# um-dsrg/Super-Resolution-Meta-Attention-Networks

Measured on AMD Instinct MI355X. Metric: LR-patches/sec (128x128x3, x4) fwd+bwd, higher is better.
Workload: dtype f32

## Files before the change

super-resolution-meta-attention-networks_amd/csrc/wgrad3x3_mfma.hip:

```cpp
#include "sisr_common.h"
#include <string.h>
#include <stdlib.h>

#define WT_H 8
#define WT_W 32
#define WH_H (WT_H + 2)
#define WH_W (WT_W + 2)
#define WSTR 32
#define X_ITEMS (WH_H * WH_W * 8)
#define X_ITERS ((X_ITEMS + 255) / 256)
#define Y_ITEMS (WT_H * WT_W * 8)
#define Y_ITERS (Y_ITEMS / 256)
#define LDS_X (WH_H * WH_W * WSTR)
#define LDS_Y (WT_H * WT_W * WSTR)
#define SLAB (9 * 16 * 64)
#define WG_MAX_UNITS 64

struct WgradParams {
  const float* x;
  View xv;
  const float* dy;
  View yv;
  const float* dy_scale;
  const float* dy_shift;
// ... 100 lines not shown
          const int ghe = h0 - 1 + er;
          if (!interior && !refl) e = sisr_keep_if(e, ghe >= 0 && ghe < H && gwe >= 0 && gwe < W);
          if (tl < 160) *reinterpret_cast<f32x4*>(ldx + er * (WH_W * WSTR) + (eside ? WH_W - 1 : 0) * WSTR + ec4 * 4) = e;
        }
      }
    }
    __syncthreads();

#pragma unroll 1
    for (int r = 2 * wave; r < 2 * wave + 2; ++r) {
      const float* xa = ldx + (r * WH_W + kk) * WSTR + i;
      const float* yb = ldy + (r * WT_W + kk) * WSTR + i;
#pragma unroll 4
      for (int u = 0; u < 16; ++u) {
        const float bv = yb[u * 2 * WSTR];
        float av[9];
#pragma unroll
        for (int t = 0; t < 9; ++t) av[t] = xa[((t / 3) * WH_W + (t % 3) + 2 * u) * WSTR];
#pragma unroll
        for (int t = 0; t < 9; ++t) acc[t] = __builtin_amdgcn_mfma_f32_32x32x2f32(av[t], bv, acc[t], 0, 0, 0);
      }
    }
  }

  __syncthreads();
  float* red = lds;
  if (wave >= 2) {
#pragma unroll
    for (int t = 0; t < 9; ++t)
#pragma unroll
      for (int r = 0; r < 16; ++r) red[(wave - 2) * SLAB + (t * 16 + r) * 64 + lane] = acc[t][r];
  }
  __syncthreads();
  if (wave < 2) {
#pragma unroll
    for (int t = 0; t < 9; ++t)
#pragma unroll
      for (int r = 0; r < 16; ++r) acc[t][r] += red[wave * SLAB + (t * 16 + r) * 64 + lane];
  }
  __syncthreads();
  if (wave == 1) {
#pragma unroll
    for (int t = 0; t < 9; ++t)
#pragma unroll
      for (int r = 0; r < 16; ++r) red[(t * 16 + r) * 64 + lane] = acc[t][r];
  }
  if (do_bias) *reinterpret_cast<f32x4*>(red + SLAB + tid * 4) = bsum;
  __syncthreads();
  if (wave == 0) {
    float* out = p.slabs + ((long)blockIdx.x * nrows + blockIdx.y) * SLAB;
#pragma unroll
    for (int t = 0; t < 9; ++t)
#pragma unroll
      for (int r = 0; r < 16; ++r) out[(t * 16 + r) * 64 + lane] = acc[t][r] + red[(t * 16 + r) * 64 + lane];
  }
  if (do_bias && tid < 32) {
    float s = 0.f;
    const int c4 = tid >> 2, e = tid & 3;
    for (int k = 0; k < 32; ++k) s += red[SLAB + (k * 8 + c4) * 4 + e];
    p.bias_slabs[((long)blockIdx.x * p.cout_chunks * 2 + cq * 2 + coh) * 32 + tid] = s;
  }
}

__global__ __launch_bounds__(256, 2) void wgrad3x3_c64_kernel(WgradParams p) { wgrad3x3_c64_body(p); }
__global__ __launch_bounds__(256, 2) void wgrad3x3_c64_geo_kernel(WgradParams p) { wgrad3x3_c64_body<true>(p); }

#define WG_BATCH 8
struct WgradBatch {
  WgradParams job[WG_BATCH];
};
__global__ __launch_bounds__(256, 2) void wgrad3x3_c64_batch_kernel(WgradBatch bt) { wgrad3x3_c64_body(bt.job[blockIdx.z]); }
__global__ __launch_bounds__(256, 2) void wgrad3x3_c64_geo_batch_kernel(WgradBatch bt) { wgrad3x3_c64_body<true>(bt.job[blockIdx.z]); }

#define FW_X (WH_H * WH_W * 64)
#define FW_Y (WT_H * WT_W * 64)

template <bool GEO = false>
static __device__ __forceinline__ void wgrad3x3_c64_full_body(const WgradParams& p) {
  extern __shared__ __attribute__((aligned(16))) float lds[];
  float* ldx = lds;
  float* ldy = lds + FW_X;
  const int tid = threadIdx.x, lane = tid & 63, wave = tid >> 6;
  const int pair = blockIdx.y;
  const int cq = pair % p.cout_chunks, cc = pair / p.cout_chunks;
  const int cih = __builtin_amdgcn_readfirstlane(wave >> 1), coh = __builtin_amdgcn_readfirstlane(wave & 1);
  const int i = lane & 31, kk = lane >> 5;
  const int H = p.H, W = p.W;
  const bool do_bias = p.bias_slabs && cc == 0;
  const bool affine = p.dy_scale != nullptr || p.dy_shift != nullptr;
  const int Cout = p.cout_chunks * 64;

  f32x16 acc[9];
#pragma unroll
  for (int t = 0; t < 9; ++t) acc[t] = (f32x16){0};
  f32x4 bsa = {0.f, 0.f, 0.f, 0.f}, bsb = bsa;

  const int tiles_per_img = p.tiles_w * p.tiles_h;
  const int total = tiles_per_img * p.B;
  int t_begin = blockIdx.x, t_end = total, t_step = p.S;
  if ((p.S & 7) == 0) {
    const int xcd = blockIdx.x & 7, idx = blockIdx.x >> 3, per = (total + 7) >> 3;
    t_begin = xcd * per + idx;
    t_end = min(total, (xcd + 1) * per);
    t_step = p.S >> 3;
  }
  struct Stage {
    f32x4 x[WH_H][2];
    f32x4 xe[2];
    f32x4 y[WT_H][2];
  };
  Stage st;
  const int c8 = tid & 7, pcol = tid >> 3;
  const int eidx = tid % 160, er = eidx >> 4, eside = (eidx >> 3) & 1, ec8 = eidx & 7;
  auto decode = [&](int tile, int& b, int& h0, int& w0) {
    b = tile / tiles_per_img;
    const int tr = tile - b * tiles_per_img;
    const int th = tr / p.tiles_w;
    h0 = th * WT_H;
    w0 = (tr - th * p.tiles_w) * WT_W;
  };
  const bool refl = GEO && p.geo_reflect;
  const int gup = GEO ? p.geo_up : 0, ysub = GEO ? p.geo_ysub : 0;
  auto xpix = [&](int g, int n) {
    if (refl) g = g < 0 ? -g : (g >= n ? 2 * n - 2 - g : g);
    return min(max(g, 0), n - 1) >> gup;
  };
  auto issue = [&](int tile) {
    int b, h0, w0;
    decode(tile, b, h0, w0);
    const sisr_rsrc_t rx = sisr_rsrc(p.x + (long)b * p.xv.sB + p.xv.chunk(cc));
    const sisr_rsrc_t ry = sisr_rsrc(p.dy + (long)b * p.yv.sB + p.yv.chunk(cq));
    const unsigned vx = (unsigned)(xpix(w0 + pcol, W) * (int)p.xv.sW + c8 * 8) * 4u;
    const unsigned vy = (unsigned)((min(w0 + pcol, W - 1) >> ysub) * (int)p.yv.sW + c8 * 8) * 4u;
#pragma unroll
    for (int r = 0; r < WH_H; ++r) {
      const unsigned so = (unsigned)(xpix(h0 - 1 + r, H) * (int)p.xv.sH) * 4u;
      st.x[r][0] = sisr_buf_load4(rx, vx, so);
      st.x[r][1] = sisr_buf_load4(rx, vx + 16u, so);
    }
    {
      const int gwe = xpix(eside ? w0 + WT_W : w0 - 1, W);
      const unsigned ve = (unsigned)(xpix(h0 - 1 + er, H) * (int)p.xv.sH + gwe * (int)p.xv.sW + ec8 * 8) * 4u;
      st.xe[0] = sisr_buf_load4(rx, ve, 0u);
      st.xe[1] = sisr_buf_load4(rx, ve + 16u, 0u);
    }
#pragma unroll
    for (int r = 0; r < WT_H; ++r) {
      const unsigned so = (unsigned)((min(h0 + r, H - 1) >> ysub) * (int)p.yv.sH) * 4u;
      st.y[r][0] = sisr_buf_load4(ry, vy, so);
      st.y[r][1] = sisr_buf_load4(ry, vy + 16u, so);
    }
  };
  auto commit = [&](int tile) {
    int b, h0, w0;
    decode(tile, b, h0, w0);
    const bool interior = !ysub && h0 >= 1 && h0 + WT_H + 1 <= H && w0 >= 1 && w0 + WT_W + 1 <= W;
    const bool okc = w0 + pcol < W;
    const bool oky = okc && !(ysub && ((w0 + pcol) & 1));
    float* lx = ldx + (pcol + 1) * 64 + c8 * 8;
    if (!interior && !refl) {
#pragma unroll
      for (int r = 0; r < WH_H; ++r) {
        const int gh = h0 - 1 + r;
        const bool ok = gh >= 0 && gh < H && okc;
        st.x[r][0] = sisr_keep_if(st.x[r][0], ok);
        st.x[r][1] = sisr_keep_if(st.x[r][1], ok);
      }
      const int gwe = eside ? w0 + WT_W : w0 - 1, ghe = h0 - 1 + er;
      const bool oke = ghe >= 0 && ghe < H && gwe >= 0 && gwe < W;
      st.xe[0] = sisr_keep_if(st.xe[0], oke);
      st.xe[1] = sisr_keep_if(st.xe[1], oke);
    }
#pragma unroll
    for (int r = 0; r < WH_H; ++r) {
      *reinterpret_cast<f32x4*>(lx + r * (WH_W * 64)) = st.x[r][0];
      *reinterpret_cast<f32x4*>(lx + r * (WH_W * 64) + 4) = st.x[r][1];
    }
    if (tid < 160) {
      float* le = ldx + (er * WH_W + (eside ? WH_W - 1 : 0)) * 64 + ec8 * 8;
      *reinterpret_cast<f32x4*>(le) = st.xe[0];
      *reinterpret_cast<f32x4*>(le + 4) = st.xe[1];
    }
    if (affine) {
      f32x4 s4a = {1.f, 1.f, 1.f, 1.f}, s4b = s4a, t4a = {0.f, 0.f, 0.f, 0.f}, t4b = t4a;
      if (p.dy_scale) {
        const float* sp = p.dy_scale + (long)b * Cout + cq * 64 + c8 * 8;
        s4a = *reinterpret_cast<const f32x4*>(sp);
        s4b = *reinterpret_cast<const f32x4*>(sp + 4);
      }
      if (p.dy_shift) {
        const float* tp = p.dy_shift + (long)b * Cout + cq * 64 + c8 * 8;
        t4a = *reinterpret_cast<const f32x4*>(tp);
        t4b = *reinterpret_cast<const f32x4*>(tp + 4);
      }
#pragma unroll
      for (int r = 0; r < WT_H; ++r) {
        st.y[r][0] = st.y[r][0] * s4a + t4a;
        st.y[r][1] = st.y[r][1] * s4b + t4b;
      }
    }
    if (!interior) {
#pragma unroll
      for (int r = 0; r < WT_H; ++r) {
        const bool ok = oky && (h0 + r < H) && !(ysub && ((h0 + r) & 1));
        st.y[r][0] = sisr_keep_if(st.y[r][0], ok);
        st.y[r][1] = sisr_keep_if(st.y[r][1], ok);
      }
    }
    float* ly = ldy + pcol * 64 + c8 * 8;
#pragma unroll
    for (int r = 0; r < WT_H; ++r) {
      *reinterpret_cast<f32x4*>(ly + r * (WT_W * 64)) = st.y[r][0];
      *reinterpret_cast<f32x4*>(ly + r * (WT_W * 64) + 4) = st.y[r][1];
    }
    if (do_bias) {
#pragma unroll
      for (int r = 0; r < WT_H; ++r) {
        bsa += st.y[r][0];
        bsb += st.y[r][1];
      }
    }
  };

  if (t_begin < t_end) {
    issue(t_begin);
    commit(t_begin);
  }
  __syncthreads();
  for (int tile = t_begin; tile < t_end; tile += t_step) {
    const bool has_next = tile + t_step < t_end;
    if (has_next) issue(tile + t_step);
    {
      const float* xa = ldx + kk * 64 + cih * 32 + i;
      const float* yb = ldy + kk * 64 + coh * 32 + i;
      float bv = yb[0], av[9];
#pragma unroll
      for (int t = 0; t < 9; ++t) av[t] = xa[((t / 3) * WH_W + (t % 3)) * 64];
#pragma unroll 1
      for (int r = 0; r < WT_H; ++r) {
        const int rn = r + 1 < WT_H ? 1 : 0;
        const float* xn = xa + rn * (WH_W * 64);
        const float* yn = yb + rn * (WT_W * 64);
#pragma unroll
        for (int u = 0; u < 16; ++u) {
          float bn, an[9];
          if (u < 15) {
            bn = yb[(u + 1) * 2 * 64];
#pragma unroll
            for (int t = 0; t < 9; ++t) an[t] = xa[((t / 3) * WH_W + (t % 3) + 2 * (u + 1)) * 64];
          } else {
            bn = yn[0];
#pragma unroll
            for (int t = 0; t < 9; ++t) an[t] = xn[((t / 3) * WH_W + (t % 3)) * 64];
          }
          __builtin_amdgcn_sched_barrier(0);
#pragma unroll
          for (int t = 0; t < 9; ++t) acc[t] = __builtin_amdgcn_mfma_f32_32x32x2f32(av[t], bv, acc[t], 0, 0, 0);
          __builtin_amdgcn_sched_barrier(0);
          bv = bn;
#pragma unroll
          for (int t = 0; t < 9; ++t) av[t] = an[t];
        }
        xa = xn;
        yb = yn;
      }
    }
    __syncthreads();
    if (has_next) {
      commit(tile + t_step);
      __syncthreads();
    }
  }

  {
    float* out = p.slabs + ((long)blockIdx.x * ((long)gridDim.y * 4) + pair * 4 + cih * 2 + coh) * SLAB;
#pragma unroll
    for (int t = 0; t < 9; ++t)
#pragma unroll
      for (int r = 0; r < 16; ++r) out[(t * 16 + r) * 64 + lane] = acc[t][r];
  }
  if (do_bias) {
    __syncthreads();
    float* red = lds;
    *reinterpret_cast<f32x4*>(red + tid * 8) = bsa;
    *reinterpret_cast<f32x4*>(red + tid * 8 + 4) = bsb;
    __syncthreads();
    if (tid < 64) {
      const int cc8 = tid >> 3, e = tid & 7;
      float s = 0.f;
      for (int k = 0; k < 32; ++k) s += red[(k * 8 + cc8) * 8 + e];
      p.bias_slabs[((long)blockIdx.x * p.cout_chunks + cq) * 64 + tid] = s;
    }
  }
}

__global__ __launch_bounds__(256, 1) void wgrad3x3_c64_full_kernel(WgradParams p) { wgrad3x3_c64_full_body(p); }
__global__ __launch_bounds__(256, 1) void wgrad3x3_c64_full_batch_kernel(WgradBatch bt) { wgrad3x3_c64_full_body(bt.job[blockIdx.z]); }
__global__ __launch_bounds__(256, 1) void wgrad3x3_c64_full_geo_kernel(WgradParams p) { wgrad3x3_c64_full_body<true>(p); }

#define W4_TH 4
#define W4_HH (W4_TH + 2)
#define W4G_X (W4_HH * WH_W * 64)
#define W4G_Y (W4_TH * WT_W * 64)
#define W4G_CHUNK (4 * 32 * 64)
#define W4G_LDS ((W4G_X + W4G_Y + 2 * W4G_CHUNK) * 4)

__global__ __launch_bounds__(256, 1) void wgrad3x3_c64_w4_kernel(WgradParams p) {
  extern __shared__ __attribute__((aligned(16))) float lds[];
  float* const ldx = lds;
  float* const ldy = lds + W4G_X;
  float* const vch = ldy + W4G_Y;
  float* const mch = vch + W4G_CHUNK;
  const int tid = threadIdx.x, lane = tid & 63, wave = tid >> 6;
  const int pair = blockIdx.y;
  const int cq = pair % p.cout_chunks, cc = pair / p.cout_chunks;
  const int cih = __builtin_amdgcn_readfirstlane(wave >> 1), coh = __builtin_amdgcn_readfirstlane(wave & 1);
  const int i = lane & 31, kk = lane >> 5;
  const int H = p.H, W = p.W;
  const bool do_bias = p.bias_slabs && cc == 0;
  const bool affine = p.dy_scale != nullptr || p.dy_shift != nullptr;
  const int Cout = p.cout_chunks * 64;

  f32x16 acc[16];
#pragma unroll
  for (int t = 0; t < 16; ++t) acc[t] = (f32x16){0};
  f32x4 bsa = {0.f, 0.f, 0.f, 0.f}, bsb = bsa;

  const int tiles_w = p.tiles_w, tiles_h = (H + W4_TH - 1) / W4_TH;
  const int tiles_per_img = tiles_w * tiles_h;
  const int total = tiles_per_img * p.B;
  int t_begin = blockIdx.x, t_end = total, t_step = p.S;
  if ((p.S & 7) == 0) {
    const int xcd = blockIdx.x & 7, idx = blockIdx.x >> 3, per = (total + 7) >> 3;
    t_begin = xcd * per + idx;
    t_end = min(total, (xcd + 1) * per);
    t_step = p.S >> 3;
  }
  struct Stage {
    f32x4 x[W4_HH][2];
    f32x4 xe[2];
    f32x4 y[W4_TH][2];
  };
  Stage st;
  const int c8 = tid & 7, pcol = tid >> 3;
  const int eidx = tid % 96, er = eidx >> 4, eside = (eidx >> 3) & 1, ec8 = eidx & 7;
  auto decode = [&](int tile, int& b, int& h0, int& w0) {
    b = tile / tiles_per_img;
    const int tr = tile - b * tiles_per_img;
    const int th = tr / tiles_w;
    h0 = th * W4_TH;
    w0 = (tr - th * tiles_w) * WT_W;
  };
  auto issue = [&](int tile) {
    int b, h0, w0;
    decode(tile, b, h0, w0);
    const sisr_rsrc_t rx = sisr_rsrc(p.x + (long)b * p.xv.sB + p.xv.chunk(cc));
    const sisr_rsrc_t ry = sisr_rsrc(p.dy + (long)b * p.yv.sB + p.yv.chunk(cq));
    const unsigned vx = (unsigned)(min(w0 + pcol, W - 1) * (int)p.xv.sW + c8 * 8) * 4u;
    const unsigned vy = (unsigned)(min(w0 + pcol, W - 1) * (int)p.yv.sW + c8 * 8) * 4u;
#pragma unroll
    for (int r = 0; r < W4_HH; ++r) {
      const unsigned so = (unsigned)(min(max(h0 - 1 + r, 0), H - 1) * (int)p.xv.sH) * 4u;
      st.x[r][0] = sisr_buf_load4(rx, vx, so);
      st.x[r][1] = sisr_buf_load4(rx, vx + 16u, so);
    }
    {
      const int gwe = min(max(eside ? w0 + WT_W : w0 - 1, 0), W - 1);
      const unsigned ve = (unsigned)(min(max(h0 - 1 + er, 0), H - 1) * (int)p.xv.sH + gwe * (int)p.xv.sW + ec8 * 8) * 4u;
      st.xe[0] = sisr_buf_load4(rx, ve, 0u);
      st.xe[1] = sisr_buf_load4(rx, ve + 16u, 0u);
    }
#pragma unroll
    for (int r = 0; r < W4_TH; ++r) {
      const unsigned so = (unsigned)(min(h0 + r, H - 1) * (int)p.yv.sH) * 4u;
      st.y[r][0] = sisr_buf_load4(ry, vy, so);
      st.y[r][1] = sisr_buf_load4(ry, vy + 16u, so);
    }
  };
  auto commit = [&](int tile) {
    int b, h0, w0;
    decode(tile, b, h0, w0);
    const bool interior = h0 >= 1 && h0 + W4_TH + 1 <= H && w0 >= 1 && w0 + WT_W + 1 <= W;
    const bool okc = w0 + pcol < W;
    if (!interior) {
#pragma unroll
      for (int r = 0; r < W4_HH; ++r) {
        const int gh = h0 - 1 + r;
        const bool ok = gh >= 0 && gh < H && okc;
        st.x[r][0] = sisr_keep_if(st.x[r][0], ok);
        st.x[r][1] = sisr_keep_if(st.x[r][1], ok);
      }
      const int gwe = eside ? w0 + WT_W : w0 - 1, ghe = h0 - 1 + er;
      const bool oke = ghe >= 0 && ghe < H && gwe >= 0 && gwe < W;
      st.xe[0] = sisr_keep_if(st.xe[0], oke);
      st.xe[1] = sisr_keep_if(st.xe[1], oke);
    }
    float* lx = ldx + (pcol + 1) * 64 + c8 * 8;
#pragma unroll
    for (int r = 0; r < W4_HH; ++r) {
      *reinterpret_cast<f32x4*>(lx + r * (WH_W * 64)) = st.x[r][0];
      *reinterpret_cast<f32x4*>(lx + r * (WH_W * 64) + 4) = st.x[r][1];
    }
    if (tid < 96) {
      float* le = ldx + (er * WH_W + (eside ? WH_W - 1 : 0)) * 64 + ec8 * 8;
      *reinterpret_cast<f32x4*>(le) = st.xe[0];
      *reinterpret_cast<f32x4*>(le + 4) = st.xe[1];
    }
    if (affine) {
      f32x4 s4a = {1.f, 1.f, 1.f, 1.f}, s4b = s4a, t4a = {0.f, 0.f, 0.f, 0.f}, t4b = t4a;
      if (p.dy_scale) {
        const float* sp = p.dy_scale + (long)b * Cout + cq * 64 + c8 * 8;
        s4a = *reinterpret_cast<const f32x4*>(sp);
        s4b = *reinterpret_cast<const f32x4*>(sp + 4);
      }
      if (p.dy_shift) {
        const float* tp = p.dy_shift + (long)b * Cout + cq * 64 + c8 * 8;
        t4a = *reinterpret_cast<const f32x4*>(tp);
        t4b = *reinterpret_cast<const f32x4*>(tp + 4);
      }
#pragma unroll
      for (int r = 0; r < W4_TH; ++r) {
        st.y[r][0] = st.y[r][0] * s4a + t4a;
        st.y[r][1] = st.y[r][1] * s4b + t4b;
      }
    }
    if (!interior) {
#pragma unroll
      for (int r = 0; r < W4_TH; ++r) {
        const bool ok = okc && h0 + r < H;
        st.y[r][0] = sisr_keep_if(st.y[r][0], ok);
        st.y[r][1] = sisr_keep_if(st.y[r][1], ok);
      }
    }
    float* ly = ldy + pcol * 64 + c8 * 8;
#pragma unroll
    for (int r = 0; r < W4_TH; ++r) {
      *reinterpret_cast<f32x4*>(ly + r * (WT_W * 64)) = st.y[r][0];
      *reinterpret_cast<f32x4*>(ly + r * (WT_W * 64) + 4) = st.y[r][1];
    }
    if (do_bias) {
#pragma unroll
      for (int r = 0; r < W4_TH; ++r) {
        bsa += st.y[r][0];
        bsb += st.y[r][1];
      }
    }
  };

  const int vb = tid >> 3, q = tid & 7;
  const int vbr = vb >> 4, vbc = vb & 15;
  auto build = [&](int xr) {
#pragma unroll
    for (int hf = 0; hf < 2; ++hf) {
      const int ch = (q + 8 * hf) * 4;
      {
        const int ra = xr == 0 ? 0 : (xr == 3 ? 3 : 2), rb = xr == 0 ? 2 : 1;
        f32x4 rr[4];
#pragma unroll
        for (int j = 0; j < 4; ++j) {
          const float* base = ldx + (2 * vbc + j) * 64 + ch;
          const f32x4 da = *reinterpret_cast<const f32x4*>(base + (2 * vbr + ra) * (WH_W * 64));
          const f32x4 db = *reinterpret_cast<const f32x4*>(base + (2 * vbr + rb) * (WH_W * 64));
          rr[j] = xr == 0 ? da - db : (xr == 1 ? db + da : (xr == 2 ? da - db : db - da));
        }
        float* vw = vch + vb * 64 + ch;
        *reinterpret_cast<f32x4*>(vw + 0 * 2048) = rr[0] - rr[2];
        *reinterpret_cast<f32x4*>(vw + 1 * 2048) = rr[1] + rr[2];
        *reinterpret_cast<f32x4*>(vw + 2 * 2048) = rr[2] - rr[1];
        *reinterpret_cast<f32x4*>(vw + 3 * 2048) = rr[1] - rr[3];
      }
      {
        f32x4 rr[2];
#pragma unroll
        for (int j = 0; j < 2; ++j) {
          const float* base = ldy + (2 * vbc + j) * 64 + ch;
          const f32x4 y0 = *reinterpret_cast<const f32x4*>(base + (2 * vbr) * (WT_W * 64));
          const f32x4 y1 = *reinterpret_cast<const f32x4*>(base + (2 * vbr + 1) * (WT_W * 64));
          rr[j] = xr == 0 ? y0 : (xr == 1 ? y0 + y1 : (xr == 2 ? y0 - y1 : y1));
        }
        float* mw = mch + vb * 64 + ch;
        *reinterpret_cast<f32x4*>(mw + 0 * 2048) = rr[0];
        *reinterpret_cast<f32x4*>(mw + 1 * 2048) = rr[0] + rr[1];
        *reinterpret_cast<f32x4*>(mw + 2 * 2048) = rr[0] - rr[1];
        *reinterpret_cast<f32x4*>(mw + 3 * 2048) = rr[1];
      }
    }
  };

  if (t_begin < t_end) {
    issue(t_begin);
    commit(t_begin);
  }
  for (int tile = t_begin; tile < t_end; tile += t_step) {
    const bool has_next = tile + t_step < t_end;
    if (has_next) issue(tile + t_step);
#pragma unroll
    for (int xr = 0; xr < 4; ++xr) {
      __syncthreads();
      build(xr);
      __syncthreads();
      if (xr == 3 && has_next) commit(tile + t_step);
      const float* va = vch + kk * 64 + cih * 32 + i;
      const float* vm = mch + kk * 64 + coh * 32 + i;
      float pa[4], pb[4];
#pragma unroll
      for (int s = 0; s < 4; ++s) {
        pa[s] = va[s * 128];
        pb[s] = vm[s * 128];
      }
#pragma unroll
      for (int s = 0; s < 64; ++s) {
        const float a = pa[s & 3], bb = pb[s & 3];
        if (s + 4 < 64) {
          pa[s & 3] = va[(s + 4) * 128];
          pb[s & 3] = vm[(s + 4) * 128];
        }
        __builtin_amdgcn_sched_barrier(0);
        acc[xr * 4 + (s >> 4)] = __builtin_amdgcn_mfma_f32_32x32x2f32(a, bb, acc[xr * 4 + (s >> 4)], 0, 0, 0);
        __builtin_amdgcn_sched_barrier(0);
      }
    }
  }

  {
    float* out = p.slabs + ((long)blockIdx.x * ((long)gridDim.y * 4) + pair * 4 + cih * 2 + coh) * SLAB;
    auto fold = [](float u0, float u1, float u2, float u3, float& f0, float& f1, float& f2) {
      const float h = 0.5f * (u1 + u2);
      f0 = u0 + h;
      f1 = 0.5f * (u1 - u2);
      f2 = h - u3;
    };
#pragma unroll
    for (int r = 0; r < 16; ++r) {
      float rw[3][4];
#pragma unroll
      for (int xc = 0; xc < 4; ++xc) fold(acc[xc][r], acc[4 + xc][r], acc[8 + xc][r], acc[12 + xc][r], rw[0][xc], rw[1][xc], rw[2][xc]);
#pragma unroll
      for (int kh = 0; kh < 3; ++kh) {
        float g0, g1, g2;
        fold(rw[kh][0], rw[kh][1], rw[kh][2], rw[kh][3], g0, g1, g2);
        out[((kh * 3 + 0) * 16 + r) * 64 + lane] = g0;
        out[((kh * 3 + 1) * 16 + r) * 64 + lane] = g1;
        out[((kh * 3 + 2) * 16 + r) * 64 + lane] = g2;
      }
    }
  }
  if (do_bias) {
    __syncthreads();
    float* red = lds;
    *reinterpret_cast<f32x4*>(red + tid * 8) = bsa;
    *reinterpret_cast<f32x4*>(red + tid * 8 + 4) = bsb;
    __syncthreads();
    if (tid < 64) {
      const int cc8 = tid >> 3, e = tid & 7;
      float s = 0.f;
      for (int k = 0; k < 32; ++k) s += red[(k * 8 + cc8) * 8 + e];
      p.bias_slabs[((long)blockIdx.x * p.cout_chunks + cq) * 64 + tid] = s;
    }
  }
}

typedef __bf16 bf16x4 __attribute__((ext_vector_type(4)));
typedef __bf16 bf16x8 __attribute__((ext_vector_type(8)));
typedef bf16x4 __attribute__((address_space(3))) * lds_bf16x4_ptr;
#define BW_PIX 128
#define BW_X_BYTES (WH_H * WH_W * BW_PIX)
#define BW_Y_BYTES (WT_H * WT_W * BW_PIX)

__device__ __forceinline__ u32x4 wg_pack_bf16x8(f32x4 a, f32x4 b) {
  bf16x8 r;
  r[0] = (__bf16)a[0]; r[1] = (__bf16)a[1]; r[2] = (__bf16)a[2]; r[3] = (__bf16)a[3];
  r[4] = (__bf16)b[0]; r[5] = (__bf16)b[1]; r[6] = (__bf16)b[2]; r[7] = (__bf16)b[3];
  return __builtin_bit_cast(u32x4, r);
}

__device__ __forceinline__ bf16x8 wg_tr_frag(const unsigned char* base, unsigned off0, unsigned off1) {
  const bf16x4 lo = __builtin_amdgcn_ds_read_tr16_b64_v4bf16((lds_bf16x4_ptr)(base + off0));
  const bf16x4 hi = __builtin_amdgcn_ds_read_tr16_b64_v4bf16((lds_bf16x4_ptr)(base + off1));
  return __builtin_shufflevector(lo, hi, 0, 1, 2, 3, 4, 5, 6, 7);
}

template <bool X16, bool Y16>
static __device__ __forceinline__ void wgrad3x3_c64_bf16_body(const WgradParams& p, unsigned* stamp = nullptr) {
  extern __shared__ __attribute__((aligned(16))) unsigned char ldsb[];
  unsigned char* ldx = ldsb;
  unsigned char* ldy = ldsb + BW_X_BYTES;
  const int tid = threadIdx.x, lane = tid & 63, wave = tid >> 6;
  const int pair = blockIdx.y;
  const int cq = pair % p.cout_chunks, cc = pair / p.cout_chunks;
  const int cih = __builtin_amdgcn_readfirstlane(wave >> 1), coh = __builtin_amdgcn_readfirstlane(wave & 1);
  const int H = p.H, W = p.W;
  const bool do_bias = p.bias_slabs && cc == 0;
  const int Cout = p.cout_chunks * 64;

  f32x16 acc[9];
#pragma unroll
  for (int t = 0; t < 9; ++t) acc[t] = (f32x16){0};
  f32x4 bsa = {0.f, 0.f, 0.f, 0.f}, bsb = bsa;

  unsigned aoff[3][2], yoff[2];
  {
    const int g = lane >> 4, qq = (lane >> 2) & 3, pp = lane & 3;
    const int chunk = (g & 1) * 2 + (pp >> 1), sub = (pp & 1) * 8;
#pragma unroll
    for (int rd = 0; rd < 2; ++rd) {
      const int pix = 8 * (g >> 1) + 4 * rd + qq;
      yoff[rd] = pix * BW_PIX + (((coh * 4 + chunk) ^ (((pix >> 1) & 1) << 2)) << 4) + sub;
#pragma unroll
      for (int kw = 0; kw < 3; ++kw)
        aoff[kw][rd] = (pix + kw) * BW_PIX + (((cih * 4 + chunk) ^ ((((pix + kw) >> 1) & 1) << 2)) << 4) + sub;
    }
  }

  const int tiles_per_img = p.tiles_w * p.tiles_h;
  const int total = tiles_per_img * p.B;
  int t_begin = blockIdx.x, t_end = total, t_step = p.S;
  if ((p.S & 7) == 0) {
    const int xcd = blockIdx.x & 7, idx = blockIdx.x >> 3, per = (total + 7) >> 3;
    t_begin = xcd * per + idx;
    t_end = min(total, (xcd + 1) * per);
    t_step = p.S >> 3;
  }
  struct Stage {
    f32x4 x[WH_H][X16 ? 1 : 2];
    f32x4 xe[X16 ? 1 : 2];
    f32x4 y[WT_H][Y16 ? 1 : 2];
  };
  Stage st;
  const int c8 = tid & 7, pcol = tid >> 3;
  const int eidx = tid % 160, er = eidx >> 4, eside = (eidx >> 3) & 1, ec8 = eidx & 7;
  auto unpack8 = [](f32x4 raw, f32x4& a, f32x4& b) {
    const u32x4 w = __builtin_bit_cast(u32x4, raw);
    a[0] = __uint_as_float(w[0] << 16); a[1] = __uint_as_float(w[0] & 0xffff0000u);
    a[2] = __uint_as_float(w[1] << 16); a[3] = __uint_as_float(w[1] & 0xffff0000u);
    b[0] = __uint_as_float(w[2] << 16); b[1] = __uint_as_float(w[2] & 0xffff0000u);
    b[2] = __uint_as_float(w[3] << 16); b[3] = __uint_as_float(w[3] & 0xffff0000u);
  };
  auto decode = [&](int tile, int& b, int& h0, int& w0) {
    b = tile / tiles_per_img;
    const int tr = tile - b * tiles_per_img;
    const int th = tr / p.tiles_w;
    h0 = th * WT_H;
    w0 = (tr - th * p.tiles_w) * WT_W;
  };
  auto issue = [&](int tile) {
    int b, h0, w0;
    decode(tile, b, h0, w0);
    const int gxi = min(w0 + pcol, W - 1) * (int)p.xv.sW + c8 * 8;
    const int gwe = min(max(eside ? w0 + WT_W : w0 - 1, 0), W - 1);
    if (X16) {
      const unsigned short* xb = reinterpret_cast<const unsigned short*>(p.x) + (long)b * p.xv.sB + p.xv.chunk(cc);
#pragma unroll
      for (int r = 0; r < WH_H; ++r)
        st.x[r][0] = *reinterpret_cast<const f32x4*>(xb + (long)min(max(h0 - 1 + r, 0), H - 1) * p.xv.sH + gxi);
      st.xe[0] = *reinterpret_cast<const f32x4*>(xb + (long)min(max(h0 - 1 + er, 0), H - 1) * p.xv.sH + gwe * (int)p.xv.sW + ec8 * 8);
    } else {
      const float* xb = p.x + (long)b * p.xv.sB + p.xv.chunk(cc);
#pragma unroll
      for (int r = 0; r < WH_H; ++r) {
        const float* a = xb + (long)min(max(h0 - 1 + r, 0), H - 1) * p.xv.sH + gxi;
        st.x[r][0] = *reinterpret_cast<const f32x4*>(a);
        st.x[r][X16 ? 0 : 1] = *reinterpret_cast<const f32x4*>(a + 4);
      }
      const float* e = xb + (long)min(max(h0 - 1 + er, 0), H - 1) * p.xv.sH + gwe * (int)p.xv.sW + ec8 * 8;
      st.xe[0] = *reinterpret_cast<const f32x4*>(e);
      st.xe[X16 ? 0 : 1] = *reinterpret_cast<const f32x4*>(e + 4);
    }
    const int gyi = min(w0 + pcol, W - 1) * (int)p.yv.sW + c8 * 8;
    if (Y16) {
      const unsigned short* yb = reinterpret_cast<const unsigned short*>(p.dy) + (long)b * p.yv.sB + p.yv.chunk(cq);
#pragma unroll
      for (int r = 0; r < WT_H; ++r) st.y[r][0] = *reinterpret_cast<const f32x4*>(yb + (long)min(h0 + r, H - 1) * p.yv.sH + gyi);
    } else {
      const float* yb = p.dy + (long)b * p.yv.sB + p.yv.chunk(cq);
#pragma unroll
      for (int r = 0; r < WT_H; ++r) {
        const float* a = yb + (long)min(h0 + r, H - 1) * p.yv.sH + gyi;
        st.y[r][0] = *reinterpret_cast<const f32x4*>(a);
        st.y[r][Y16 ? 0 : 1] = *reinterpret_cast<const f32x4*>(a + 4);
      }
    }
  };
  auto commit = [&](int tile) {
    int b, h0, w0;
    decode(tile, b, h0, w0);
    const int col = pcol + 1;
    const bool cokx = w0 + pcol < W;
    const unsigned lx = col * BW_PIX + ((c8 ^ (((col >> 1) & 1) << 2)) << 4);
#pragma unroll
    for (int r = 0; r < WH_H; ++r) {
      const int gh = h0 - 1 + r;
      u32x4 pk = X16 ? __builtin_bit_cast(u32x4, st.x[r][0]) : wg_pack_bf16x8(st.x[r][0], st.x[r][X16 ? 0 : 1]);
      const unsigned m = (gh >= 0 && gh < H && cokx) ? 0xffffffffu : 0u;
      pk &= (u32x4){m, m, m, m};
      *reinterpret_cast<u32x4*>(ldx + r * (WH_W * BW_PIX) + lx) = pk;
    }
    {
      const int ecol = eside ? WH_W - 1 : 0, gwe = eside ? w0 + WT_W : w0 - 1, ghe = h0 - 1 + er;
      u32x4 pk = X16 ? __builtin_bit_cast(u32x4, st.xe[0]) : wg_pack_bf16x8(st.xe[0], st.xe[X16 ? 0 : 1]);
      const unsigned m = (ghe >= 0 && ghe < H && gwe >= 0 && gwe < W) ? 0xffffffffu : 0u;
      pk &= (u32x4){m, m, m, m};
      if (tid < 160)
        *reinterpret_cast<u32x4*>(ldx + er * (WH_W * BW_PIX) + ecol * BW_PIX + ((ec8 ^ (((ecol >> 1) & 1) << 2)) << 4)) = pk;
    }
    f32x4 s4a = {1.f, 1.f, 1.f, 1.f}, s4b = s4a, t4a = {0.f, 0.f, 0.f, 0.f}, t4b = t4a;
    if (p.dy_scale) {
      const float* sp = p.dy_scale + (long)b * Cout + cq * 64 + c8 * 8;
      s4a = *reinterpret_cast<const f32x4*>(sp);
      s4b = *reinterpret_cast<const f32x4*>(sp + 4);
    }
    if (p.dy_shift) {
      const float* tp = p.dy_shift + (long)b * Cout + cq * 64 + c8 * 8;
      t4a = *reinterpret_cast<const f32x4*>(tp);
      t4b = *reinterpret_cast<const f32x4*>(tp + 4);
    }
    const bool coky = w0 + pcol < W;
    const unsigned ly = pcol * BW_PIX + ((c8 ^ (((pcol >> 1) & 1) << 2)) << 4);
#pragma unroll
    for (int r = 0; r < WT_H; ++r) {
      const bool ok = coky && (h0 + r < H);
      f32x4 ya, yb2;
      if (Y16) unpack8(st.y[r][0], ya, yb2);
      else { ya = st.y[r][0]; yb2 = st.y[r][Y16 ? 0 : 1]; }
      const f32x4 ta = sisr_keep_if(ya * s4a + t4a, ok), tb = sisr_keep_if(yb2 * s4b + t4b, ok);
      bsa += ta;
      bsb += tb;
      *reinterpret_cast<u32x4*>(ldy + r * (WT_W * BW_PIX) + ly) = wg_pack_bf16x8(ta, tb);
    }
  };

  unsigned long long st_life = 0, st_a = 0, st_k = 0, st_c = 0;
  unsigned st_tiles = 0;
  if (stamp) st_life = __builtin_amdgcn_s_memtime();
  if (t_begin < t_end) {
    issue(t_begin);
    commit(t_begin);
  }
  __syncthreads();
  for (int tile = t_begin; tile < t_end; tile += t_step) {
    const bool has_next = tile + t_step < t_end;
    if (stamp) st_a = __builtin_amdgcn_s_memtime();
    if (has_next) issue(tile + t_step);

    {
      bf16x8 af[2][9], bf[2];
      auto load_step = [&](int ks, bf16x8* a9, bf16x8& b1) {
        const int r = ks >> 1, hf = ks & 1;
        b1 = wg_tr_frag(ldy + (r * WT_W + 16 * hf) * BW_PIX, yoff[0], yoff[1]);
#pragma unroll
        for (int t = 0; t < 9; ++t)
          a9[t] = wg_tr_frag(ldx + ((r + t / 3) * WH_W + 16 * hf) * BW_PIX, aoff[t % 3][0], aoff[t % 3][1]);
      };
      load_step(0, af[0], bf[0]);
#pragma unroll
      for (int ks = 0; ks < 2 * WT_H; ++ks) {
        if (ks + 1 < 2 * WT_H) load_step(ks + 1, af[(ks + 1) & 1], bf[(ks + 1) & 1]);
#pragma unroll
        for (int t = 0; t < 9; ++t)
          acc[t] = __builtin_amdgcn_mfma_f32_32x32x16_bf16(af[ks & 1][t], bf[ks & 1], acc[t], 0, 0, 0);
        __builtin_amdgcn_sched_barrier(0);
      }
    }
    if (stamp) {
      const unsigned long long t = __builtin_amdgcn_s_memtime();
      st_k += t - st_a;
      st_a = t;
      ++st_tiles;
    }
    __syncthreads();
    if (has_next) {
      commit(tile + t_step);
      __syncthreads();
    }
    if (stamp) st_c += __builtin_amdgcn_s_memtime() - st_a;
  }
  if (stamp && lane == 0) {
    unsigned* dbg = stamp + ((long)(blockIdx.y * gridDim.x + blockIdx.x) * 4 + wave) * 8;
    dbg[0] = (unsigned)(__builtin_amdgcn_s_memtime() - st_life);
    dbg[1] = (unsigned)st_k;
    dbg[2] = 0;
    dbg[3] = (unsigned)st_c;
    dbg[4] = st_tiles;
    dbg[5] = __builtin_amdgcn_s_getreg(4 | (31 << 11));
    dbg[6] = __builtin_amdgcn_s_getreg(20 | (31 << 11));
    dbg[7] = (unsigned)(st_life & 0xffffffffu);
  }

  {
    float* out = p.slabs + ((long)blockIdx.x * ((long)gridDim.y * 4) + pair * 4 + cih * 2 + coh) * SLAB;
#pragma unroll
    for (int t = 0; t < 9; ++t)
#pragma unroll
      for (int r = 0; r < 16; ++r) out[(t * 16 + r) * 64 + lane] = acc[t][r];
  }
  if (do_bias) {
    __syncthreads();
    float* red = reinterpret_cast<float*>(ldsb);
    *reinterpret_cast<f32x4*>(red + tid * 8) = bsa;
    *reinterpret_cast<f32x4*>(red + tid * 8 + 4) = bsb;
    __syncthreads();
    if (tid < 64) {
      const int c8 = tid >> 3, e = tid & 7;
      float s = 0.f;
      for (int k = 0; k < 32; ++k) s += red[(k * 8 + c8) * 8 + e];
      p.bias_slabs[((long)blockIdx.x * p.cout_chunks + cq) * 64 + tid] = s;
    }
  }
}
__global__ __launch_bounds__(256, 1) void wgrad3x3_c64_bf16_kernel(WgradParams p) { wgrad3x3_c64_bf16_body<false, false>(p); }
__global__ __launch_bounds__(256, 1) void wgrad3x3_c64_bf16_x16_kernel(WgradParams p) { wgrad3x3_c64_bf16_body<true, false>(p); }
__global__ __launch_bounds__(256, 1) void wgrad3x3_c64_bf16_xy16_kernel(WgradParams p) { wgrad3x3_c64_bf16_body<true, true>(p); }
#ifdef SISR_DIAG
static unsigned* g_diag_wgrad_stamp = nullptr;
extern "C" void sisr_diag_wgrad_stamp(void* buf) { g_diag_wgrad_stamp = static_cast<unsigned*>(buf); }
__global__ __launch_bounds__(256, 1) void wgrad3x3_c64_bf16_xy16_stamp_kernel(WgradParams p, unsigned* stamp) {
  wgrad3x3_c64_bf16_body<true, true>(p, stamp);
}
#endif

#define XW_TH 4
#define XW_HH (XW_TH + 2)
#define XW_X (XW_HH * WH_W * BW_PIX)
// ... 889 lines not shown
```

Baseline: 115.2.

## Compute Winograd transforms in registers and software-pipeline them with MFMA

Drops the LDS staging buffers for the transformed input and gradient chunks in the w4 wgrad kernel. Each lane now fetches raw values straight from the tile in LDS and applies the Winograd transforms in registers, double-buffered across k-steps. Scheduling group barriers interleave MFMAs with LDS reads and VALU work. This removes the per-xr build passes and their barriers, and reduces LDS footprint, at the cost of more register pressure and redundant transform arithmetic per lane.

Measured after the change: 119.1, median of 6. 1.03x the previous value.

```diff
diff --git a/super-resolution-meta-attention-networks_amd/csrc/wgrad3x3_mfma.hip b/super-resolution-meta-attention-networks_amd/csrc/wgrad3x3_mfma.hip
--- a/super-resolution-meta-attention-networks_amd/csrc/wgrad3x3_mfma.hip
+++ b/super-resolution-meta-attention-networks_amd/csrc/wgrad3x3_mfma.hip
@@ -426,15 +426,12 @@
 #define W4_HH (W4_TH + 2)
 #define W4G_X (W4_HH * WH_W * 64)
 #define W4G_Y (W4_TH * WT_W * 64)
-#define W4G_CHUNK (4 * 32 * 64)
-#define W4G_LDS ((W4G_X + W4G_Y + 2 * W4G_CHUNK) * 4)
+#define W4G_LDS ((W4G_X + W4G_Y) * 4)
 
 __global__ __launch_bounds__(256, 1) void wgrad3x3_c64_w4_kernel(WgradParams p) {
   extern __shared__ __attribute__((aligned(16))) float lds[];
   float* const ldx = lds;
   float* const ldy = lds + W4G_X;
-  float* const vch = ldy + W4G_Y;
-  float* const mch = vch + W4G_CHUNK;
   const int tid = threadIdx.x, lane = tid & 63, wave = tid >> 6;
   const int pair = blockIdx.y;
   const int cq = pair % p.cout_chunks, cc = pair / p.cout_chunks;
@@ -571,77 +568,111 @@
     }
   };
 
-  const int vb = tid >> 3, q = tid & 7;
-  const int vbr = vb >> 4, vbc = vb & 15;
-  auto build = [&](int xr) {
-#pragma unroll
-    for (int hf = 0; hf < 2; ++hf) {
-      const int ch = (q + 8 * hf) * 4;
-      {
-        const int ra = xr == 0 ? 0 : (xr == 3 ? 3 : 2), rb = xr == 0 ? 2 : 1;
-        f32x4 rr[4];
-#pragma unroll
-        for (int j = 0; j < 4; ++j) {
-          const float* base = ldx + (2 * vbc + j) * 64 + ch;
-          const f32x4 da = *reinterpret_cast<const f32x4*>(base + (2 * vbr + ra) * (WH_W * 64));
-          const f32x4 db = *reinterpret_cast<const f32x4*>(base + (2 * vbr + rb) * (WH_W * 64));
-          rr[j] = xr == 0 ? da - db : (xr == 1 ? db + da : (xr == 2 ? da - db : db - da));
-        }
-        float* vw = vch + vb * 64 + ch;
-        *reinterpret_cast<f32x4*>(vw + 0 * 2048) = rr[0] - rr[2];
-        *reinterpret_cast<f32x4*>(vw + 1 * 2048) = rr[1] + rr[2];
-        *reinterpret_cast<f32x4*>(vw + 2 * 2048) = rr[2] - rr[1];
-        *reinterpret_cast<f32x4*>(vw + 3 * 2048) = rr[1] - rr[3];
-      }
-      {
-        f32x4 rr[2];
-#pragma unroll
-        for (int j = 0; j < 2; ++j) {
-          const float* base = ldy + (2 * vbc + j) * 64 + ch;
-          const f32x4 y0 = *reinterpret_cast<const f32x4*>(base + (2 * vbr) * (WT_W * 64));
-          const f32x4 y1 = *reinterpret_cast<const f32x4*>(base + (2 * vbr + 1) * (WT_W * 64));
-          rr[j] = xr == 0 ? y0 : (xr == 1 ? y0 + y1 : (xr == 2 ? y0 - y1 : y1));
-        }
-        float* mw = mch + vb * 64 + ch;
-        *reinterpret_cast<f32x4*>(mw + 0 * 2048) = rr[0];
-        *reinterpret_cast<f32x4*>(mw + 1 * 2048) = rr[0] + rr[1];
-        *reinterpret_cast<f32x4*>(mw + 2 * 2048) = rr[0] - rr[1];
-        *reinterpret_cast<f32x4*>(mw + 3 * 2048) = rr[1];
-      }
-    }
-  };
-
+  const float* const xl = ldx + kk * (2 * 64) + cih * 32 + i;
+  const float* const yl = ldy + kk * (2 * 64) + coh * 32 + i;
+  struct Raw {
+    float d[4][4], y[2][2];
+  };
+  auto fetch = [&](int ks, Raw& rw) {
+    const int br = ks >> 3, bc = ks & 7;
+#pragma unroll
+    for (int r = 0; r < 4; ++r)
+#pragma unroll
+      for (int j = 0; j < 4; ++j) rw.d[r][j] = xl[((2 * br + r) * WH_W + 4 * bc + j) * 64];
+#pragma unroll
+    for (int r = 0; r < 2; ++r)
+#pragma unroll
+      for (int j = 0; j < 2; ++j) rw.y[r][j] = yl[((2 * br + r) * WT_W + 4 * bc + j) * 64];
+  };
+  auto transform = [&](const Raw& rw, float (&V)[16], float (&M)[16]) {
+    float rr[4][4];
+#pragma unroll
+    for (int j = 0; j < 4; ++j) {
+      rr[0][j] = rw.d[0][j] - rw.d[2][j];
+      rr[1][j] = rw.d[1][j] + rw.d[2][j];
+      rr[2][j] = rw.d[2][j] - rw.d[1][j];
+      rr[3][j] = rw.d[1][j] - rw.d[3][j];
+    }
+#pragma unroll
+    for (int xr = 0; xr < 4; ++xr) {
+      V[xr * 4 + 0] = rr[xr][0] - rr[xr][2];
+      V[xr * 4 + 1] = rr[xr][1] + rr[xr][2];
+      V[xr * 4 + 2] = rr[xr][2] - rr[xr][1];
+      V[xr * 4 + 3] = rr[xr][1] - rr[xr][3];
+    }
+    float ry[4][2];
+#pragma unroll
+    for (int j = 0; j < 2; ++j) {
+      ry[0][j] = rw.y[0][j];
+      ry[1][j] = rw.y[0][j] + rw.y[1][j];
+      ry[2][j] = rw.y[0][j] - rw.y[1][j];
+      ry[3][j] = rw.y[1][j];
+    }
+#pragma unroll
+    for (int xr = 0; xr < 4; ++xr) {
+      M[xr * 4 + 0] = ry[xr][0];
+      M[xr * 4 + 1] = ry[xr][0] + ry[xr][1];
+      M[xr * 4 + 2] = ry[xr][0] - ry[xr][1];
+      M[xr * 4 + 3] = ry[xr][1];
+    }
+  };
+
+  float V[2][16], M[2][16];
+  auto step_order = [&]() {
+#pragma unroll
+    for (int t = 0; t < 2; ++t) {
+      __builtin_amdgcn_sched_group_barrier(0x008, 1, 0);
+      __builtin_amdgcn_sched_group_barrier(0x100, 5, 0);
+    }
+    __builtin_amdgcn_sched_group_barrier(0x008, 2, 0);
+#pragma unroll
+    for (int t = 4; t < 15; ++t) {
+      __builtin_amdgcn_sched_group_barrier(0x008, 1, 0);
+      __builtin_amdgcn_sched_group_barrier(0x002, 4, 0);
+    }
+    __builtin_amdgcn_sched_group_barrier(0x008, 1, 0);
+  };
   if (t_begin < t_end) {
     issue(t_begin);
     commit(t_begin);
+    __syncthreads();
+    Raw rw;
+    fetch(0, rw);
+    transform(rw, V[0], M[0]);
   }
   for (int tile = t_begin; tile < t_end; tile += t_step) {
     const bool has_next = tile + t_step < t_end;
     if (has_next) issue(tile + t_step);
 #pragma unroll
-    for (int xr = 0; xr < 4; ++xr) {
-      __syncthreads();
-      build(xr);
-      __syncthreads();
-      if (xr == 3 && has_next) commit(tile + t_step);
-      const float* va = vch + kk * 64 + cih * 32 + i;
-      const float* vm = mch + kk * 64 + coh * 32 + i;
-      float pa[4], pb[4];
-#pragma unroll
-      for (int s = 0; s < 4; ++s) {
-        pa[s] = va[s * 128];
-        pb[s] = vm[s * 128];
-      }
-#pragma unroll
-      for (int s = 0; s < 64; ++s) {
-        const float a = pa[s & 3], bb = pb[s & 3];
-        if (s + 4 < 64) {
-          pa[s & 3] = va[(s + 4) * 128];
-          pb[s & 3] = vm[(s + 4) * 128];
-        }
-        __builtin_amdgcn_sched_barrier(0);
-        acc[xr * 4 + (s >> 4)] = __builtin_amdgcn_mfma_f32_32x32x2f32(a, bb, acc[xr * 4 + (s >> 4)], 0, 0, 0);
-        __builtin_amdgcn_sched_barrier(0);
+    for (int ks = 0; ks < 15; ++ks) {
+      const int cur = ks & 1, nxt = cur ^ 1;
+      Raw rw;
+      fetch(ks + 1, rw);
+#pragma unroll
+      for (int t = 0; t < 16; ++t)
+        acc[t] = __builtin_amdgcn_mfma_f32_32x32x2f32(V[cur][t], M[cur][t], acc[t], 0, 0, 0);
+      transform(rw, V[nxt], M[nxt]);
+      step_order();
+    }
+    __syncthreads();
+    if (has_next) commit(tile + t_step);
+#pragma unroll
+    for (int t = 0; t < 8; ++t) acc[t] = __builtin_amdgcn_mfma_f32_32x32x2f32(V[1][t], M[1][t], acc[t], 0, 0, 0);
+    __builtin_amdgcn_sched_barrier(0);
+    __syncthreads();
+    {
+      Raw rw;
+      fetch(0, rw);
+#pragma unroll
+      for (int t = 8; t < 16; ++t) acc[t] = __builtin_amdgcn_mfma_f32_32x32x2f32(V[1][t], M[1][t], acc[t], 0, 0, 0);
+      transform(rw, V[0], M[0]);
+      __builtin_amdgcn_sched_group_barrier(0x008, 1, 0);
+      __builtin_amdgcn_sched_group_barrier(0x100, 10, 0);
+      __builtin_amdgcn_sched_group_barrier(0x008, 2, 0);
+#pragma unroll
+      for (int t = 0; t < 5; ++t) {
+        __builtin_amdgcn_sched_group_barrier(0x008, 1, 0);
+        __builtin_amdgcn_sched_group_barrier(0x002, 9, 0);
       }
     }
   }
```
